# wagnva/semantic-nerf-for-satellite-data

Measured on AMD Instinct MI355X. Metric: train rays/sec (4096 rays x 64 samples), higher is better.
Workload: dtype f32(f16x2)

## Files before the change

### semantic-nerf-for-satellite-data_amd/csrc/api.hip

```cpp
#include <stdarg.h>
#include <stdio.h>
#include <stdlib.h>
#include <string.h>

#include <mutex>

#include "aux_kernels.h"
#include "bsp.h"
#include "composite.h"
#include "gemm.h"
#include "plan.h"

namespace snerf {

int forward_bsp(const Plan& p, const float* pk, const SnerfInputs* in, const SnerfOutputs* out, void* workspace, hipStream_t st);
int backward_bsp(const Plan& p, const float* pk, const SnerfInputs* in, const SnerfOutGrads* go, float* gp, float* d_t, float* d_t_s,
                 void* workspace, hipStream_t st);

static thread_local char g_err[512] = "";
void set_error(const char* fmt, ...) {
  va_list ap;
  va_start(ap, fmt);
  vsnprintf(g_err, sizeof(g_err), fmt, ap);
  va_end(ap);
// ... 179 lines not shown
    p.k_tr[i] = (i == 0) ? p.Ep : (((p.skip_mask >> i) & 1u) ? p.Ep + p.W : p.W);
    p.w_tr[i] = take((size_t)p.W * p.k_tr[i]);
    p.b_tr[i] = take(p.W);
  }
  p.w_fs = take((size_t)(p.W + NARROW) * p.W); p.b_fs = take(p.W + NARROW);
  p.w_h1 = take((size_t)p.N1 * p.FA); p.b_h1 = take(p.N1);
  p.w_s2 = take((size_t)p.H * p.H); p.b_s2 = take(p.H);
  p.w_s3 = take((size_t)p.H * p.H); p.b_s3 = take(p.H);
  p.w_s4 = take((size_t)NARROW * p.H); p.b_s4 = take(NARROW);
  p.w_fin = take((size_t)NARROW * p.KF); p.b_fin = take(NARROW);
  p.sky_floats = 9 * p.H + 4;
  p.sky = take(p.sky_floats);
  p.n_fp32 = off;
  {
    const char* ev = getenv("SNERF_COMPOSE_FEATS");
    p.compose_feats = p.pl == 2 && (p.H & 31) == 0 && p.N1 + NARROW <= 2048 && !(ev && ev[0] == '0' && ev[1] == 0);
  }
  if (!p.compose_feats) { plan_weights(p); plan_bsp(p); return SNERF_OK; }
  Plan q = p;
  q.compose_feats = false;
  plan_weights(q);
  plan_bsp(q);
  plan_weights(p);
  plan_bsp(p);
  if (q.packed_floats > p.packed_floats) p.packed_floats = q.packed_floats;
  if (q.ws_bytes > p.ws_bytes) p.ws_bytes = q.ws_bytes;
  return SNERF_OK;
}

struct TableBuilder {
  CopyTable tabs[4];
  int nt = 0;
  bool missing = false;
  TableBuilder() { memset(tabs, 0, sizeof(tabs)); nt = 1; }
  void add(float* user, int user_ld, int rows, int cols, size_t dst_off, int dst_ld) {
    if (!user) { missing = true; return; }
    if (tabs[nt - 1].n == COPY_TABLE_MAX) ++nt;
    CopyEntry& e = tabs[nt - 1].e[tabs[nt - 1].n++];
    e.user = user; e.user_ld = user_ld; e.rows = rows; e.cols = cols; e.dst_off = dst_off; e.dst_ld = dst_ld;
  }
};

static void build_tables(const Plan& p, const SnerfParams* w, TableBuilder& tb) {
  const int W = p.W, H = p.H, E = p.E;
  for (int i = 0; i < p.L; ++i) {
    const bool skip = (p.skip_mask >> i) & 1u;
    if (i == 0) {
// ... 195 lines not shown
```

### semantic-nerf-for-satellite-data_amd/csrc/aux_kernels.h

```cpp
#pragma once
#include "common.h"
#include "../../include/snerf_hip.h"

namespace snerf {

struct EncodeArgs {
  const float* rays = nullptr;
  const float* xyz = nullptr;
  const float* z = nullptr;
  const float* sun_d = nullptr; int sun_stride = 3;
  const float* t = nullptr; const float* t_s = nullptr;
  int dir_is_sun = 0;
  int N = 0, S = 0, F = 0, Ep = 0;
  int FA = 0, W = 0, Xp = 0, x_sun = 0, x_t = 3, x_ts = -1, tau = 0;
  unsigned* zero = nullptr; int zero_n = 0;
};

struct CopyEntry {
  float* user; int user_ld; int rows; int cols; unsigned long long dst_off; int dst_ld;
};
constexpr int COPY_TABLE_MAX = 40;
struct CopyTable { CopyEntry e[COPY_TABLE_MAX]; int n; };

int launch_zero_bytes(void* p, size_t bytes, hipStream_t st);
int launch_sample_z(const float* rays, const float* zsteps, const float* u, float* z, int N, int S, hipStream_t st);
int launch_copy_table(const CopyTable& tb, float* packed, int mode, hipStream_t st);
int launch_reduce_rows(const float* in, int n_in, size_t in_stride, int width, float* out, size_t out_stride,
                       int group, int accumulate, hipStream_t st);
int reduce_partials(const float* in, int n_in, size_t in_stride, int width, float* tmp, float* out, hipStream_t st);
struct RedJob { const float* in; float* out; unsigned long long stride; long long width; int n_in; int blk0; int vec; int cols; int in_ld; int out_ld; int store; int pad; };
constexpr int RED_MAX = 56;
struct RedTable { RedJob j[RED_MAX]; int n = 0; int blocks = 0; };
constexpr int RED_CHUNK = 24;
struct RedChunk { RedJob j[RED_CHUNK]; int n = 0; };
int red_add_elem(RedTable& tb, const float* in, int n_in, size_t stride, size_t width, float* out);
int red_add_elem2d(RedTable& tb, const float* in, int n_in, size_t stride, int rows, int cols, int in_ld, float* out, int out_ld);
int red_add_col(RedTable& tb, const float* in, int n_in, size_t stride, int width, float* out);
int red_store_last(RedTable& tb);
int launch_reductions(const RedTable& elem, const RedTable& col, hipStream_t st);
// ... 6 lines not shown
```

### semantic-nerf-for-satellite-data_amd/csrc/bsp.h

```cpp
#pragma once
#include "common.h"
#include "gemm.h"

namespace snerf {
namespace bsp {

constexpr int RB = 128;
constexpr int CB = 128;
constexpr int E_MAX = 100;
constexpr int E_QUIET = 60;

typedef __amdgpu_buffer_rsrc_t srd_t;
typedef unsigned int u32x4 __attribute__((ext_vector_type(4)));
typedef unsigned int u32x2 __attribute__((ext_vector_type(2)));
typedef _Float16 f16x8 __attribute__((ext_vector_type(8)));
typedef _Float16 f16x4 __attribute__((ext_vector_type(4)));
constexpr unsigned OOB = 0xFFFFFFF0u;

__host__ __device__ inline int ncb_of(int ld) { return (ld + CB - 1) / CB; }
__host__ __device__ inline size_t plane_bytes(size_t rows, int ld, int pl = 2) { return rows * (size_t)ld * 2 * pl; }
__host__ __device__ inline size_t etab_ints(size_t rows, int ld) { return ((rows + RB - 1) / RB) * (size_t)ncb_of(ld); }
__host__ __device__ inline unsigned g16_off(int k, int pl = 2) { return (unsigned)(k >> 4) * 32u * (unsigned)pl + (unsigned)(k & 15) * 2u; }

__host__ __device__ inline int exp_of_maxbits(unsigned b) {
// ... 65 lines not shown
  int Ka = 0;
  const char* W = nullptr;
  const int* EW = nullptr;
  int w_rb32 = 0, w_row0 = 0, w_k0 = 0; unsigned w_bytes = 0;
  int I = 0, J = 0, K = 0;
  char* C = nullptr; int* EC = nullptr; int ldc = 0; int c_col0 = 0;
  float* Cf = nullptr;
  const float* bias = nullptr;
  int act = ACT_NONE; float w0 = 1.f;
  unsigned* Csign = nullptr;
  int aux_mode = AUX_NONE;
  const char* H = nullptr; const int* EH = nullptr; int ldh = 0; int h_col0 = 0; const unsigned* Hsign = nullptr;
  float* colsum = nullptr; int ldcs = 0;
  int tiles_i = 0, tiles_j = 0;
  int tj_skip = -1;
  int tiles_jr = 0;
  int rev = 0;
  int dbg = 0;
  int* tile_ctr = nullptr;
  int pl = 2;
  const float* nd_w = nullptr; float* nd_out = nullptr; unsigned long long nd_stride = 0;
  int nd_omax = 0, nd_ldw = 0;
  int nd_rows[8] = {0, 0, 0, 0, 0, 0, 0, 0}, nd_row0[8] = {0, 0, 0, 0, 0, 0, 0, 0}, nd_woff[8] = {0, 0, 0, 0, 0, 0, 0, 0};
};
__host__ __device__ inline size_t sign_words(size_t rows, int ld) { return ((rows + 31) / 32) * (size_t)((ld + 63) / 64) * 64; }

struct DwArgs {
  const char* A = nullptr; const int* EA = nullptr; int lda = 0; int a_col0 = 0;
  const char* B = nullptr; const int* EB = nullptr; int ldb = 0; int b_col0 = 0;
  int I = 0, J = 0, P = 0;
  float* C = nullptr; int ldc = 0;
  int k_split = 0, n_split = 1; unsigned long long slab_stride = 0;
  int tiles_i = 0, tiles_j = 0;
  int pl = 2;
};

constexpr int TR_MAXL = 8;
constexpr int TR_SLOTS = TR_MAXL + 1;
struct TrunkArgs {
  const char* pe = nullptr; const int* Epe = nullptr;
  int P = 0, W = 0, L = 0; unsigned skip_mask = 0;
  int gamma_free_layer = 0;
  const char* Wp[TR_SLOTS] = {}; const int* EW[TR_SLOTS] = {}; unsigned w_bytes[TR_SLOTS] = {}; int K[TR_SLOTS] = {};
  const float* bias[TR_SLOTS] = {}; float w0[TR_SLOTS] = {};
  char* F = nullptr; int* EF = nullptr; int ldf = 0;
  char* H[TR_MAXL] = {}; int* EH[TR_MAXL] = {}; unsigned* Hsign[TR_MAXL] = {};
// ... 68 lines not shown
```

### semantic-nerf-for-satellite-data_amd/csrc/bsp_aux.hip

```cpp
#include "bsp.h"
#include "aux_kernels.h"

namespace snerf {
namespace bsp {

__device__ __forceinline__ float block_max_256(float m, float* sm) {
#pragma unroll
  for (int o = 32; o >= 1; o >>= 1) m = fmaxf(m, __shfl_xor(m, o, 64));
  __syncthreads();
  if ((threadIdx.x & 63) == 0) sm[threadIdx.x >> 6] = m;
  __syncthreads();
  return fmaxf(fmaxf(sm[0], sm[1]), fmaxf(sm[2], sm[3]));
}

__global__ __launch_bounds__(256) void to_planes_kernel(const float* __restrict__ src, int ld_src, int rows, int cols,
                                                        char* __restrict__ dst, int* __restrict__ E, int ld, int col0, int pl) {
  __shared__ float sm[4];
  const int rb = blockIdx.y, cb = blockIdx.x;
  const int t = threadIdx.x, c8 = cb * 128 + (t & 15) * 8;
  float v[8][8];
  float m = 0.f;
#pragma unroll
  for (int i = 0; i < 8; ++i) {
    const int r = rb * 128 + (t >> 4) + 16 * i;
// ... 319 lines not shown
#pragma unroll
    for (int half = 0; half < 2; ++half) {
#pragma unroll
      for (int j = 0; j < 8; ++j) h8[j] = v[8 * half + j];
      split8(h8, sc, hi, lo);
      *reinterpret_cast<u32x4*>(d + 16 * half) = hi;
      if (g.pl == 2) *reinterpret_cast<u32x4*>(d + 32 + 16 * half) = lo;
    }
  }
}

int launch_encode_bsp(const EncodeArgs& a, char* pe, int* Epe, char* fa, int* Efa, int fa_col0, int pl, hipStream_t st) {
  if (a.Ep > 128 || (a.Ep & 15) || (fa && ((fa_col0 & 127) || (a.FA & 15) || a.Xp != 16))) {
    set_error("encode: Ep <= 128, Ep % 16 == 0, extras block of 16 columns at a multiple of 128");
    return SNERF_ERR_BAD_DESC;
  }
  EncodeBsp g{a, pe, Epe, fa, Efa, fa_col0, pl};
  const long long P = (long long)a.N * a.S;
  hipLaunchKernelGGL(encode_bsp_kernel, dim3((unsigned)((P + 127) / 128)), dim3(256), 0, st, g);
  SNERF_LAUNCH_CHECK();
  return SNERF_OK;
}

__global__ __launch_bounds__(256) void colsum32_bsp_kernel(const float* __restrict__ in, int rows, float* __restrict__ partial,
                                                           char* __restrict__ pl, int* __restrict__ E, int npl) {
  __shared__ float4 sm[32][8];
  __shared__ float smx[2][2];
  const int c4 = threadIdx.x & 7, rg = threadIdx.x >> 3;
  const int r0 = blockIdx.x * 256;
  float4 v[8];
  float4 s = make_float4(0.f, 0.f, 0.f, 0.f);
  float m[2] = {0.f, 0.f};
#pragma unroll
  for (int i = 0; i < 8; ++i) {
    const int r = r0 + rg + 32 * i;
    v[i] = r < rows ? *reinterpret_cast<const float4*>(in + (size_t)r * 32 + 4 * c4) : make_float4(0.f, 0.f, 0.f, 0.f);
    s.x += v[i].x; s.y += v[i].y; s.z += v[i].z; s.w += v[i].w;
    m[i >> 2] = fmaxf(fmaxf(m[i >> 2], fmaxf(fabsf(v[i].x), fabsf(v[i].y))), fmaxf(fabsf(v[i].z), fabsf(v[i].w)));
  }
  sm[rg][c4] = s;
#pragma unroll
  for (int h = 0; h < 2; ++h) {
#pragma unroll
    for (int o = 32; o >= 1; o >>= 1) m[h] = fmaxf(m[h], __shfl_xor(m[h], o, 64));
  }
  __syncthreads();
// ... 44 lines not shown
```

### semantic-nerf-for-satellite-data_amd/csrc/bsp_kc.hip

```cpp
#include "bsp_kc_epi.h"

namespace snerf {
namespace bsp {

constexpr int KC_A = 128 * 128, KC_RING = 3;
constexpr int KC_RINGB = KC_RING * KC_A;
constexpr int KC_XREG = KC_RINGB;
constexpr int KC_BIAS = KC_XREG + 4 * 4096;
constexpr int KC_ETAB = KC_BIAS + 2 * 1024;
constexpr int KC_SMAX = KC_ETAB + 2 * 512;
constexpr int KC_NEXT = KC_SMAX + 64;
constexpr int KC_HSIGN = KC_NEXT + 64;
constexpr int KC_LDS = KC_HSIGN + 4 * 1024;
constexpr int KC_NDW = KC_HSIGN;
constexpr int KC_NDW_FLOATS = 2560;
constexpr int KC_LDS_ND = KC_NDW + 4 * KC_NDW_FLOATS;
template <int PL, int ACT, int AUX, bool COLSUM, bool SIGNS, int SINM, bool DIAG = false, int NDOT = 0>
__global__ __launch_bounds__(256, 2) void gemm_kc_kernel(const KcArgs) {
  const kargs_t p = kargs();
  __shared__ __attribute__((aligned(16))) char lds[NDOT > 0 ? KC_LDS_ND : KC_LDS];
  float* smax = reinterpret_cast<float*>(lds + KC_SMAX);
  const int t = threadIdx.x, lane = t & 63;
  const int wave = __builtin_amdgcn_readfirstlane(t >> 6);
  const int wj0 = wave * 64;
  const int tiles_i = p->tiles_i, tiles_j = p->tiles_j, ntiles = tiles_i * tiles_j;
  constexpr int EB = 2 * PL;
  constexpr int KSUB = PL == 2 ? 16 : 32, KSH = PL == 2 ? 4 : 5;
  const int nks16 = p->K >> 4;
  const int nks = (p->K + KSUB - 1) >> KSH;
  const int nks1 = p->Ka < p->K ? p->Ka >> KSH : nks;
  const int eW = *p->EW;
  const int nst = (nks + 1) >> 1, nst1 = nks1 >> 1;
  constexpr bool ONEPASS = ACT == ACT_SIN;
  constexpr bool BIAS = AUX == AUX_NONE && !COLSUM;
  const int dbg = DIAG ? p->dbg : 0;

  auto a_lane_off = [&](int q, int ld, int l) -> unsigned {
    const int row = 8 * (wave + 4 * q) + (l >> 3);
    return (unsigned)row * (unsigned)ld * (unsigned)EB + 16u * (unsigned)((l & 7) ^ ((row >> 1) & 7));
  };
// ... 400 lines not shown
      if (AUX == AUX_SINREC) {
        const srd_words srdS = make_srd_words(e->Hsign, clamp_bytes(sign_words((size_t)e->I, e->ldh) * 4ull));
        const unsigned sreg0 = __builtin_amdgcn_readfirstlane(lds_addr(lds + KC_HSIGN + wave * 1024));
#pragma unroll
        for (int mi = 0; mi < 4; ++mi) {
          const bool ok = wave_cols && 32 * mi < nrows;
          const unsigned vo = ok ? (unsigned)((((size_t)((c_i0 >> 5) + mi) * ((e->ldh + 63) >> 6) + ((e->h_col0 + jw) >> 6)) * 64 + el) * 4) : OOBH;
          dma4_asm(srdS, sreg0 + (unsigned)(mi * 256), vo, 0u);
        }
      }
      dma_h(0);
      dma_h(1);
      if constexpr (AUX != AUX_NONE) next_heads();
      const float fac = AUX == AUX_SINREC ? inv_in * fabsf(e->w0) * inv_h : inv_in;
      const int eHc = eH < -60 ? -60 : (eH > 60 ? 60 : eH);
      const float one_s = pow2f(2 * eHc);
      const unsigned sflip = e->w0 < 0.f ? 0xFFFFFFFFu : 0u;
      unsigned sword[4] = {0u, 0u, 0u, 0u};
#pragma unroll
      for (int nj = 0; nj < 2; ++nj) {
        float cs[16];
#pragma unroll
        for (int r = 0; r < 16; ++r) cs[r] = 0.f;
#pragma unroll
        for (int mi = 0; mi < 4; ++mi) {
          const int hb = 4 * nj + mi;
          u32x4 hh[2], hl[2];
          if (AUX != AUX_NONE) {
            if (hb == 7) wait_vm<0>(); else if (hb < 2 && more) wait_vm<HPC + 8>(); else wait_vm<HPC>();
            const char* hreg = (hb & 1) ? lds + KC_XREG + wave * 4096 : lds + 2 * KC_A + wave * 4096;
            if (AUX == AUX_SINREC && nj == 0) sword[mi] = *reinterpret_cast<const unsigned*>(lds + KC_HSIGN + wave * 1024 + mi * 256 + el * 4) ^ sflip;
#pragma unroll
            for (int gg = 0; gg < 2; ++gg) {
              if constexpr (PL == 2) {
                hh[gg] = *reinterpret_cast<const u32x4*>(hreg + pt * 128 + 16 * ((4 * gg + lh) ^ ((pt >> 1) & 7)));
                if (AUX == AUX_SINREC) hl[gg] = *reinterpret_cast<const u32x4*>(hreg + pt * 128 + 16 * ((4 * gg + 2 + lh) ^ ((pt >> 1) & 7)));
              } else {
                hh[gg] = *reinterpret_cast<const u32x4*>(hreg + pt * 64 + 16 * ((2 * gg + lh) ^ ((pt >> 2) & 3)));
              }
            }
            if (hb + 2 < 8) {
              if constexpr (PL == 2 && AUX == AUX_SINREC) asm volatile("s_waitcnt lgkmcnt(0)" : "+v"(hh[0]), "+v"(hh[1]), "+v"(hl[0]), "+v"(hl[1]), "+v"(sword[mi])::"memory");
              else asm volatile("s_waitcnt lgkmcnt(0)" : "+v"(hh[0]), "+v"(hh[1]), "+v"(sword[mi])::"memory");
              dma_h(hb + 2);
            }
          }
// ... 16 lines not shown
#pragma unroll
              for (int c = 0; c < 8; ++c) {
                const float om = fmaf(-sv[c], sv[c], one_s);
                const float root = __builtin_amdgcn_sqrtf(fabsf(om));
                const unsigned rs = __float_as_uint(root) | ((sword[mi] << (31 - (16 * nj + 8 * gg + c))) & 0x80000000u);
                v[c] *= __uint_as_float(rs);
              }
            } else if (AUX == AUX_RELU_MASK) {
              float hv[8];
              cvt8f(hh[gg], hv);
#pragma unroll
              for (int c = 0; c < 8; ++c) v[c] = hv[c] > 0.f ? v[c] : 0.f;
            }
#pragma unroll
            for (int c = 0; c < 8; ++c) {
              if (COLSUM) cs[8 * gg + c] += v[c];
              acc[mi][nj][8 * gg + c] = v[c];
            }
            if (jw + 16 * gq < e->J) {
              const float m8 = absmax3(v[6], v[7], absmax3(v[4], v[5], absmax3(v[2], v[3], absmax3(v[0], v[1], 0.f))));
              wmax = fmaxf(wmax, (BIAS && (32 * mi + pt) >= nrows) ? 0.f : m8);
            }
          }
        }
        if (COLSUM && e->colsum != nullptr) {
#pragma unroll
          for (int r = 0; r < 16; ++r) cs[r] = sum32(cs[r]);
          if ((el & 31) == 31) {
#pragma unroll
            for (int gg = 0; gg < 2; ++gg)
              if (jw + 16 * (2 * nj + gg) < e->J) {
                float* d = e->colsum + (size_t)c_ti * e->ldcs + jw + 16 * (2 * nj + gg) + 8 * lh;
                *reinterpret_cast<float4*>(d) = make_float4(cs[8 * gg] * fac, cs[8 * gg + 1] * fac, cs[8 * gg + 2] * fac, cs[8 * gg + 3] * fac);
                *reinterpret_cast<float4*>(d + 4) = make_float4(cs[8 * gg + 4] * fac, cs[8 * gg + 5] * fac, cs[8 * gg + 6] * fac, cs[8 * gg + 7] * fac);
              }
          }
        }
      }
      constexpr bool RAW = AUX != AUX_NONE || COLSUM;
      wmax = wave_max(wmax) * (RAW ? fac : 1.f);
      if (el == 0) smax[wave] = wmax;
      barrier_raw();
      const float bmax = fmaxf(smax[wave & 2], smax[(wave & 2) + 1]);
      const int eC = exp_of_maxbits(__float_as_uint(bmax));
      const float sc = pow2f(eC) * (RAW ? fac : 1.f);
      if ((wave & 1) == 0 && el == 0 && wave_cols) e->EC[(size_t)c_ti * ncb_of(e->ldc) + ((e->c_col0 + jw) >> 7)] = eC;
      if (more) headW();
#pragma unroll
// ... 39 lines not shown
static int g_kc_grid_override = 0;
void kc_set_grid_override(int n) { g_kc_grid_override = n > 0 ? n : 0; }
static int kc_slots() {
  if (g_kc_grid_override > 0) return g_kc_grid_override;
  static const int n = [] {
    int dev = 0, cus = 256;
    if (hipGetDevice(&dev) != hipSuccess || hipDeviceGetAttribute(&cus, hipDeviceAttributeMultiprocessorCount, dev) != hipSuccess || cus <= 0) cus = 256;
    return 2 * cus;
  }();
  return n;
}

static bool cs_bias_check(const KcArgs& a) {
  if (a.colsum != nullptr && a.bias != nullptr) { set_error("bsp gemm: bias and column sums in one launch"); return true; }
  return false;
}

int launch_kc(const KcArgs& a0, hipStream_t st) {
  KcArgs a = a0;
  if (!a.A2) { a.A2 = a.A; a.EA2 = a.EA; a.lda2 = a.lda; a.a2_col0 = a.a_col0; if (a.Ka == 0) a.Ka = a.K; }
  int rc = check_kc(a, false);
  if (rc) return rc;
  if (cs_bias_check(a)) return SNERF_ERR_BAD_DESC;
  a.tiles_i = (a.I + 127) / 128;
  a.tiles_jr = (a.J + 255) / 256;
  if (a.tj_skip >= a.tiles_jr || (a.tj_skip >= 0 && a.tiles_jr < 2)) { set_error("bsp gemm: tj_skip beyond the column tiles"); return SNERF_ERR_BAD_DESC; }
  a.tiles_j = a.tiles_jr - (a.tj_skip >= 0 ? 1 : 0);
  if (a.nd_w != nullptr) {
    if (a.nd_omax == 0) { a.nd_omax = 1; a.nd_ldw = 0; for (int tj = 0; tj < 8; ++tj) { a.nd_rows[tj] = tj < a.tiles_jr ? 1 : 0; a.nd_row0[tj] = 0; } }
    int off = 0;
    for (int tj = 0; tj < a.tiles_jr && tj < 8; ++tj) { a.nd_woff[tj] = off; off += 256 * a.nd_rows[tj]; }
    if (a.tiles_jr > 8 || off > KC_NDW_FLOATS || (a.nd_omax != 1 && a.nd_omax != 5)) { set_error("bsp gemm: folded projections beyond the LDS table"); return SNERF_ERR_BAD_DESC; }
    for (int tj = 0; tj < a.tiles_jr; ++tj) if (a.nd_rows[tj] > a.nd_omax) { set_error("bsp gemm: nd_rows > nd_omax"); return SNERF_ERR_BAD_DESC; }
  }
#ifdef KC_DIAG_BUILD
  constexpr bool DIAG = true;
  static const int dbg = [] { const char* e = getenv("SNERF_KC_DBG"); return e ? atoi(e) : 0; }();
  a.dbg = dbg;
  if (dbg & 2) a.w_bytes = 0;
#else
  constexpr bool DIAG = false;
#endif
  const int ntiles = a.tiles_i * a.tiles_j, slots = kc_slots();
  const dim3 grid(ntiles < slots ? ntiles : slots), block(256);
  const int tok = prof_hook_begin(2.0 * a.I * (double)a.J * a.K, 0, st);
  const bool cs = a.colsum != nullptr;
#define KC_LAUNCH(ACT_, AUX_, CS_, SG_, SM_) do { if (a.pl == 2) hipLaunchKernelGGL((gemm_kc_kernel<2, ACT_, AUX_, CS_, SG_, SM_, DIAG>), grid, block, 0, st, a); \
                                                 else hipLaunchKernelGGL((gemm_kc_kernel<1, ACT_, AUX_, CS_, SG_, SM_, DIAG>), grid, block, 0, st, a); } while (0)
#define KC_LAUNCH_ND(SG_, ND_) do { if (a.pl == 2) hipLaunchKernelGGL((gemm_kc_kernel<2, ACT_SIN, AUX_NONE, false, SG_, SIN_DIRECT, DIAG, ND_>), grid, block, 0, st, a); \
                                    else hipLaunchKernelGGL((gemm_kc_kernel<1, ACT_SIN, AUX_NONE, false, SG_, SIN_DIRECT, DIAG, ND_>), grid, block, 0, st, a); } while (0)
  if (a.aux_mode == AUX_SINREC) KC_LAUNCH(ACT_NONE, AUX_SINREC, true, false, SIN_FRACT);
  else if (a.aux_mode == AUX_RELU_MASK) KC_LAUNCH(ACT_NONE, AUX_RELU_MASK, true, false, SIN_FRACT);
  else if (a.act == ACT_SIN) {
    if (a.nd_w != nullptr && a.nd_omax == 1) { if (a.Csign == nullptr) KC_LAUNCH_ND(false, 1); else KC_LAUNCH_ND(true, 1); }
    else if (a.nd_w != nullptr) { if (a.Csign == nullptr) KC_LAUNCH_ND(false, 5); else KC_LAUNCH_ND(true, 5); }
    else if (a.Csign == nullptr) KC_LAUNCH(ACT_SIN, AUX_NONE, false, false, SIN_DIRECT);
    else KC_LAUNCH(ACT_SIN, AUX_NONE, false, true, SIN_DIRECT);
  }
  else if (a.act == ACT_RELU) KC_LAUNCH(ACT_RELU, AUX_NONE, false, false, SIN_FRACT);
  else if (cs) KC_LAUNCH(ACT_NONE, AUX_NONE, true, false, SIN_FRACT);
  else KC_LAUNCH(ACT_NONE, AUX_NONE, false, false, SIN_FRACT);
#undef KC_LAUNCH
#undef KC_LAUNCH_ND
  SNERF_LAUNCH_CHECK();
  prof_hook_end(tok, st);
  return SNERF_OK;
}

}
}
```

### semantic-nerf-for-satellite-data_amd/csrc/bsp_pass.hip

```cpp
#include "aux_kernels.h"
#include "bsp.h"
#include "composite.h"
#include "plan.h"

namespace snerf {

namespace {
struct Ws {
  char* base;
  char* c(size_t off) const { return base + off; }
  float* f(size_t off) const { return reinterpret_cast<float*>(base + off); }
  int* i(size_t off) const { return reinterpret_cast<int*>(base + off); }
  unsigned* u(size_t off) const { return reinterpret_cast<unsigned*>(base + off); }
  void a(bsp::KcArgs& g, const PlaneT& t, int k, int col0 = 0) const { g.A = c(t.o); g.EA = i(t.e); g.lda = t.ld; g.a_col0 = col0; g.Ka = k; }
  void a2(bsp::KcArgs& g, const PlaneT& t) const { g.A2 = c(t.o); g.EA2 = i(t.e); g.lda2 = t.ld; }
  void out(bsp::KcArgs& g, const PlaneT& t, int col0 = 0) const { g.C = c(t.o); g.EC = i(t.e); g.ldc = t.ld; g.c_col0 = col0; g.Csign = t.s ? u(t.s) : nullptr; }
  void h(bsp::KcArgs& g, const PlaneT& t, int col0 = 0) const { g.H = c(t.o); g.EH = i(t.e); g.ldh = t.ld; g.h_col0 = col0; g.Hsign = t.s ? u(t.s) : nullptr; }
  void dz(bsp::DwArgs& g, const PlaneT& t) const { g.A = c(t.o); g.EA = i(t.e); g.lda = t.ld; g.a_col0 = 0; }
  void x(bsp::DwArgs& g, const PlaneT& t, int col0) const { g.B = c(t.o); g.EB = i(t.e); g.ldb = t.ld; g.b_col0 = col0; }
};
struct WOp { const char* W; const int* EW; int rb32; unsigned bytes; int K; };
WOp wop(const Plan& p, const float* pk, int job) {
  const char* planes = reinterpret_cast<const char*>(pk + p.n_fp32);
  const bsp::WPackJob& w = p.wj.j[job];
// ... 133 lines not shown
  if (p.train) { c.save_T = ws.f(p.o_T); c.save_rgbraw = ws.f(p.o_rgbraw); }
  RC(launch_composite_fwd(c, st));
  return SNERF_OK;
}

namespace {
struct RQ {
  float* base; size_t cap, used = 0; bool over = false;
  RedTable elem, col;
  float* take(size_t floats) {
    const size_t n = round_up_sz(floats, 64);
    if (used + n > cap) { over = true; return base; }
    float* r = base ? base + used : nullptr; used += n; return r;
  }
};
struct DwMat { DwSplit sp; size_t stride; int ldw; float* slab; };
inline int cs_ld(int width) { return (width + 3) & ~3; }

struct BwdRegions {
  float *nar_fin = nullptr, *nar_sun = nullptr, *nar_sig = nullptr;
  DwMat w_fin, w_s4, w_s3, w_s2, w_h1, w_fs;
  float *cs_fin = nullptr, *cs_s3 = nullptr, *cs_s2 = nullptr, *cs_sun = nullptr, *cs_fa = nullptr, *cs_hl = nullptr;
  int ld_cs1 = 0;
  struct Layer { DwMat w, w_gamma; float* cs; } tr[SNERF_MAX_LAYERS];
};
void take_regions(const Plan& p, RQ& rq, BwdRegions& r) {
  auto dw = [&](int rows, int ldw, int cols, bool narrow_rows, int split_rows = 0) {
    DwMat m;
    m.sp = dw_choose_bsp(p.P, split_rows > 0 ? split_rows : rows, cols, narrow_rows);
    m.stride = round_up_sz((size_t)rows * ldw, 64);
    m.ldw = ldw;
    m.slab = rq.take(m.stride * m.sp.ns);
    return m;
  };
  auto cs = [&](int width) { return rq.take((size_t)((p.P + 127) / 128) * cs_ld(width)); };
  auto nar = [&]() { return rq.take((size_t)((p.P + 255) / 256) * NARROW); };
  const int W = p.W, H = p.H;
  if (!p.sc) { r.nar_fin = nar(); r.w_fin = dw(NARROW, p.KF, p.KF, true); if (!p.compose_feats) r.cs_fin = cs(p.KF); }
  r.nar_sun = nar(); r.w_s4 = dw(NARROW, H, H, true); r.w_s3 = dw(H, H, H, false); r.w_s2 = dw(H, H, H, false);
  r.cs_s3 = cs(H); r.cs_s2 = cs(H);
  if (p.compose_feats) {
    r.ld_cs1 = cs_ld(p.h1w); r.cs_fin = cs(p.h1w); r.cs_sun = r.cs_fin + (p.sc ? 0 : p.sun_col);
    r.w_h1 = dw(p.h1w, p.FA, p.FA, false);
    r.nar_sig = nar(); r.w_fs = dw(NARROW, W, W, false, W); r.cs_hl = cs(W);
  } else {
    r.cs_sun = cs(H);
    r.w_h1 = dw(p.h1w, p.FA, p.FA, false); r.cs_fa = cs(p.FA);
    r.nar_sig = nar(); r.w_fs = dw(W + NARROW, W, W, false, W); r.cs_hl = cs(W);
  }
  for (int i = p.L - 1; i >= 0; --i) {
    if (i > 0 && ((p.skip_mask >> i) & 1u)) { r.tr[i].w_gamma = dw(W, p.Ep, p.Ep, false); r.tr[i].w = dw(W, W, W, false); }
    else r.tr[i].w = dw(W, p.k_tr[i], i == 0 ? p.Ep : W, false);
    r.tr[i].cs = i > 0 ? cs(W) : nullptr;
  }
}
}

size_t bsp_rq_floats(const Plan& p) {
  RQ rq{nullptr, ~(size_t)0};
  BwdRegions r;
  take_regions(p, rq, r);
  return rq.used;
}

int backward_bsp(const Plan& p, const float* pk, const SnerfInputs* in, const SnerfOutGrads* go, float* gp, float* d_t, float* d_t_s,
                 void* workspace, hipStream_t st) {
// ... 34 lines not shown
  c.sun_d = in->sun_d; c.sun_stride = in->sun_stride; c.sky = pk + p.sky;
  b.T = ws.f(p.o_T); b.rgbraw = ws.f(p.o_rgbraw);
  b.g_rgb = go->rgb; b.g_depth = go->depth; b.g_weights = go->weights; b.g_transparency = go->transparency;
  b.g_albedo = go->albedo; b.g_sun = go->sun; b.g_sky = go->sky; b.g_beta = go->beta; b.g_sigmas = go->sigmas;
  b.g_beta_s = go->beta_semantic; b.g_logits = go->semantic_logits;
  b.d_sigo = dsig; b.d_fino = dfin; b.d_suno = dsun; b.sky_slab = p.sc ? nullptr : ws.f(p.o_skyslab);
  b.zero = ws.u(p.o_kcq); b.zero_n = KCQ_SLOTS * 16;
  RC(launch_composite_bwd(b, st));
  if (!p.sc)
    RC(red_add_col(rq.col, ws.f(p.o_skyslab), p.comp_blocks * 4, (size_t)p.sky_floats, p.sky_floats, gp + p.sky));


  const PlaneT dz1 = p.dza.view(p.h1w);
  const int sun_col = p.sc ? 0 : p.sun_col;
  if (!p.sc) {
    RC(narrow_grad(dfin, r.nar_fin, p.pdfin, gp + p.b_fin));
    RC(dw_gemm(r.w_fin, p.pdfin, NARROW, true, p.h1, 0, p.KF));
    RC(dw_reduce(r.w_fin, (size_t)NARROW * p.KF, gp + p.w_fin));
    bsp::KcArgs g;
    ws.a(g, p.pdfin, NARROW); weights(g, p, pk, p.wj_tfin);
    g.I = P; g.J = p.KF; g.K = NARROW; ws.out(g, dz1);
    dact(g, p.h1);
    colsum(g, r.cs_fin, p.KF);
    if (p.compose_feats) g.ldcs = r.ld_cs1;
    RC(launch_kc(g));
    if (!p.compose_feats) RC(bias_from_colsum(r.cs_fin, p.KF, gp + p.b_h1));
  }
  {
    RC(narrow_grad(dsun, r.nar_sun, p.pdsun, gp + p.b_s4));
    RC(dw_gemm(r.w_s4, p.pdsun, NARROW, true, p.s3, 0, H));
    RC(dw_reduce(r.w_s4, (size_t)NARROW * H, gp + p.w_s4));
    bsp::KcArgs g;
    ws.a(g, p.pdsun, NARROW); weights(g, p, pk, p.wj_ts4);
    g.I = P; g.J = H; g.K = NARROW; ws.out(g, p.dsa);
    dact(g, p.s3);
    colsum(g, r.cs_s3, H);
    RC(launch_kc(g));
    RC(bias_from_colsum(r.cs_s3, H, gp + p.b_s3));
    RC(dw_gemm(r.w_s3, p.dsa, H, false, p.s2, 0, H));
    RC(dw_reduce(r.w_s3, (size_t)H * H, gp + p.w_s3));
    ws.a(g, p.dsa, H); g.K = H; weights(g, p, pk, p.wj_ts3);
    ws.out(g, p.dsb);
    dact(g, p.s2);
    colsum(g, r.cs_s2, H);
    RC(launch_kc(g));
    RC(bias_from_colsum(r.cs_s2, H, gp + p.b_s2));
    RC(dw_gemm(r.w_s2, p.dsb, H, false, p.h1, sun_col, H));
    RC(dw_reduce(r.w_s2, (size_t)H * H, gp + p.w_s2));
    ws.a(g, p.dsb, H); weights(g, p, pk, p.wj_ts2);
    ws.out(g, dz1, sun_col);
    dact(g, p.h1, sun_col);
    colsum(g, r.cs_sun, H);
    if (p.compose_feats) g.ldcs = r.ld_cs1;
    RC(launch_kc(g));
    if (!p.compose_feats) RC(bias_from_colsum(r.cs_sun, H, gp + p.b_h1 + (size_t)p.sun_col));
  }
  auto transient_grads = [&]() {
    const bool want_t = d_t != nullptr, want_ts = d_t_s != nullptr && p.x_ts >= 0;
    if (p.sc) {
      if (want_t) RC(launch_zero_bytes(d_t, (size_t)p.N * p.tau * sizeof(float), st));
      if (want_ts) RC(launch_zero_bytes(d_t_s, (size_t)p.N * p.tau * sizeof(float), st));
    } else if (want_t || want_ts) {
      int b_lo = p.blk_beta, b_hi = p.blk_beta;
      auto use = [&](int blk, bool on) { if (on && blk >= 0) { if (blk < b_lo) b_lo = blk; if (blk > b_hi) b_hi = blk; } };
      use(p.blk_rgb, p.rgb_t); use(p.blk_sem, p.sem_t || p.sem_ts); use(p.blk_sbeta, true);
      const int k_lo = b_lo * H, k_n = (b_hi + 1 - b_lo) * H;
      float* dext = ws.f(p.o_dfin);
      bsp::KcArgs x;
      ws.a(x, dz1, k_n, k_lo); weights(x, p, pk, p.wj_th1, p.Wf, k_lo);
      x.I = P; x.J = p.Xp; x.K = k_n; x.Cf = dext;
      RC(bsp::launch_kc_narrow(x, st));
      if (want_t) RC(launch_ray_sum32(dext, p.x_t, p.N, p.S, p.tau, d_t, st));
      if (want_ts) RC(launch_ray_sum32(dext, p.x_ts, p.N, p.S, p.tau, d_t_s, st));
    }
    return (int)SNERF_OK;
  };
  PlaneT dz_cur = p.dza.view(W);
  PlaneT dz_nxt = p.dzb.view(W);
  const bool sig_live = !p.sc || go->weights != nullptr || go->transparency != nullptr || go->sigmas != nullptr;
  const PlaneT& hl = p.h[p.L - 1];
  bool uncompose = false;
  if (p.compose_feats) {
    const int r0 = p.sc ? p.sun_col : 0;
    const int nt = (P + 127) / 128, X = p.FA - W;
    RC(dw_gemm(r.w_h1, dz1, p.h1w, false, p.fa, 0, p.FA));
    RC(red_add_elem2d(rq.elem, r.w_h1.slab + W, r.w_h1.sp.ns, r.w_h1.stride, p.h1w, X, p.FA, gp + p.w_h1 + (size_t)r0 * p.FA + W, p.FA));
    RC(red_add_elem2d(rq.elem, r.w_h1.slab, r.w_h1.sp.ns, r.w_h1.stride, p.h1w, W, p.FA, r.w_h1.slab, p.FA));
    RC(red_store_last(rq.elem));
    RC(red_add_col(rq.col, r.cs_fin, nt, (size_t)r.ld_cs1, p.h1w, r.cs_fin));
    RC(red_store_last(rq.col));
    uncompose = true;
    RC(transient_grads());
    if (sig_live) {
      RC(narrow_grad(dsig, r.nar_sig, p.pdsig, gp + p.b_fs + W));
      RC(dw_gemm(r.w_fs, p.pdsig, NARROW, true, hl, 0, W));
      RC(dw_reduce(r.w_fs, (size_t)NARROW * W, gp + p.w_fs + (size_t)W * W));
    }
    { const PlaneT sw = dz_cur; dz_cur = dz_nxt; dz_nxt = sw; }
    bsp::KcArgs g;
    ws.a(g, dz1, p.h1w);
    if (sig_live) ws.a2(g, p.pdsig);
    weights(g, p, pk, p.wj_th1, 0, r0); g.I = P; g.J = W; g.K = sig_live ? p.h1w + NARROW : p.h1w;
    ws.out(g, dz_cur);
    dact(g, hl, 0, (p.L == 1) ? 30.f : 1.f);
    colsum(g, r.cs_hl, W);
    RC(launch_kc(g));
    RC(bias_from_colsum(r.cs_hl, W, gp + p.b_tr[p.L - 1]));
  }
  const PlaneT dfa = p.dzb.view(p.FA);
  if (!p.compose_feats) {
    const int r0 = p.sc ? p.sun_col : 0;
    RC(dw_gemm(r.w_h1, dz1, p.h1w, false, p.fa, 0, p.FA));
    RC(dw_reduce(r.w_h1, (size_t)p.h1w * p.FA, gp + p.w_h1 + (size_t)r0 * p.FA));
// ... 58 lines not shown
```

### semantic-nerf-for-satellite-data_amd/csrc/plan.h

```cpp
#pragma once
#include "bsp.h"
#include "common.h"
#include "../../include/snerf_hip.h"

namespace snerf {

constexpr int NARROW = 32;
constexpr int MAX_CLASSES = 16;
constexpr int ND_FIN = 5;
constexpr int MAX_SKY_UNITS = 8;

struct PlaneT { size_t o = 0, e = 0, s = 0; int ld = 0; };
struct PlaneScratch {
  size_t o = 0, e = 0; int maxw = 0;
  PlaneT view(int ld) const { PlaneT t; t.o = o; t.e = e; t.ld = ld; return t; }
};

struct Plan {
  int N = 0, S = 0, P = 0, Pp = 0;
  int W = 0, H = 0, L = 0, E = 0, Ep = 0, F = 0, tau = 0, C = 0;
  bool siren = false, train = false, sc = false, sem_sigmoid = false;
  unsigned skip_mask = 0;
  int x_sun = 0, x_t = 3, x_ts = -1, Xp = 0, FA = 0;
  int nblk = 0, blk_rgb = 0, blk_sem = -1, blk_beta = -1, blk_sbeta = -1, blk_sun = -1;
// ... 17 lines not shown
  size_t packed_floats = 0;
  int pl = 2;

  size_t o_z = 0, o_T = 0, o_rgbraw = 0;
  PlaneT pe, fa, h1, s2, s3, h[SNERF_MAX_LAYERS];
  size_t o_sigo = 0, o_fino = 0, o_suno = 0;
  size_t o_sigpart = 0, o_sunpart = 0, o_finpart = 0;
  bool nd_sig = false, nd_sun = false;
  bool fuse_trunk = false;
  bool nd_fin = false;
  PlaneScratch dza, dzb;
  PlaneT dsa, dsb, pdsig, pdfin, pdsun;
  size_t o_dsig = 0, o_dfin = 0, o_dsun = 0;
  size_t o_skyslab = 0;
  size_t o_kcq = 0;
  size_t o_rq = 0, rq_floats = 0;
  bsp::WPackTable wj = {};
  int wj_tr[SNERF_MAX_LAYERS] = {0}, wj_tt[SNERF_MAX_LAYERS] = {0};
  int wj_fs = 0, wj_sig = 0, wj_tfs = 0, wj_h1 = 0, wj_th1 = 0, wj_s2 = 0, wj_ts2 = 0, wj_s3 = 0, wj_ts3 = 0, wj_s4 = 0, wj_ts4 = 0,
      wj_fin = 0, wj_tfin = 0;
  size_t wp_bytes = 0;
  int h1w = 0;
  bool compose_feats = false;
  int wj_first = 0;
  size_t o_wc = 0;
  size_t o_bc = 0;
  int comp_blocks = 0;
  size_t ws_bytes = 0;
};

constexpr int KCQ_SLOTS = 64;
struct DwSplit { int ns = 1; int k_split = 32; };
DwSplit dw_choose_bsp(int P, int rows, int cols, bool narrow_rows);

#define RC(expr) do { int _rc = (expr); if (_rc) return _rc; } while (0)

int make_plan(const SnerfDesc* d, Plan* pl);

size_t bsp_rq_floats(const Plan& p);

}
```

Before: 170,600.

## Compute per-ray extras weight grads and transient grads from per-block column sums

Adds a ray_extras path. The backward GEMM epilogue emits per-32-row column sums (one row per ray, since S is a multiple of 32), and a new kernel uses these per-ray sums to build the weight gradient for the per-ray extra input columns (sun direction, transient embeddings). The same kernel also produces the transient embedding gradients, which replaces both the wide dW GEMM over those columns and the separate transient GEMM. It relies on the extra inputs being constant within a ray, and it adds workspace, a new kernel and extra column-sum stores. The path falls back when it would need more workspace.

New measurement: 171,600 (median of 6 runs). Within noise of the previous version (+0.6%).

```diff
diff --git a/semantic-nerf-for-satellite-data_amd/csrc/api.hip b/semantic-nerf-for-satellite-data_amd/csrc/api.hip
--- a/semantic-nerf-for-satellite-data_amd/csrc/api.hip
+++ b/semantic-nerf-for-satellite-data_amd/csrc/api.hip
@@ -225,7 +225,12 @@
   plan_weights(q);
   plan_bsp(q);
   plan_weights(p);
+  {
+    const char* ev = getenv("SNERF_RAY_EXTRAS");
+    p.ray_extras = (p.S & 31) == 0 && !(ev && ev[0] == '0' && ev[1] == 0);
+  }
   plan_bsp(p);
+  if (p.ray_extras && p.ws_bytes > q.ws_bytes) { p.ray_extras = false; plan_bsp(p); }
   if (q.packed_floats > p.packed_floats) p.packed_floats = q.packed_floats;
   if (q.ws_bytes > p.ws_bytes) p.ws_bytes = q.ws_bytes;
   return SNERF_OK;
diff --git a/semantic-nerf-for-satellite-data_amd/csrc/aux_kernels.h b/semantic-nerf-for-satellite-data_amd/csrc/aux_kernels.h
--- a/semantic-nerf-for-satellite-data_amd/csrc/aux_kernels.h
+++ b/semantic-nerf-for-satellite-data_amd/csrc/aux_kernels.h
@@ -15,6 +15,22 @@
   int FA = 0, W = 0, Xp = 0, x_sun = 0, x_t = 3, x_ts = -1, tau = 0;
   unsigned* zero = nullptr; int zero_n = 0;
 };
+
+struct RayExtrasArgs {
+  EncodeArgs a;
+  const float* Q = nullptr; int ldq = 0;
+  int h1w = 0;
+  const float* Wx = nullptr; int ldw = 0;
+  int k_lo = 0, k_n = 0;
+  float* slab = nullptr;
+  float* gsum = nullptr;
+  float* part = nullptr;
+  int rays_per_group = 0;
+};
+namespace bsp {
+void ray_extras_grid(int N, int h1w, int& groups, int& rays_per_group, int& chunks);
+int launch_ray_extras(const RayExtrasArgs& a, hipStream_t st);
+}
 
 struct CopyEntry {
   float* user; int user_ld; int rows; int cols; unsigned long long dst_off; int dst_ld;
diff --git a/semantic-nerf-for-satellite-data_amd/csrc/bsp.h b/semantic-nerf-for-satellite-data_amd/csrc/bsp.h
--- a/semantic-nerf-for-satellite-data_amd/csrc/bsp.h
+++ b/semantic-nerf-for-satellite-data_amd/csrc/bsp.h
@@ -111,6 +111,7 @@
   const float* nd_w = nullptr; float* nd_out = nullptr; unsigned long long nd_stride = 0;
   int nd_omax = 0, nd_ldw = 0;
   int nd_rows[8] = {0, 0, 0, 0, 0, 0, 0, 0}, nd_row0[8] = {0, 0, 0, 0, 0, 0, 0, 0}, nd_woff[8] = {0, 0, 0, 0, 0, 0, 0, 0};
+  int cs32 = 0;
 };
 __host__ __device__ inline size_t sign_words(size_t rows, int ld) { return ((rows + 31) / 32) * (size_t)((ld + 63) / 64) * 64; }
 
diff --git a/semantic-nerf-for-satellite-data_amd/csrc/bsp_aux.hip b/semantic-nerf-for-satellite-data_amd/csrc/bsp_aux.hip
--- a/semantic-nerf-for-satellite-data_amd/csrc/bsp_aux.hip
+++ b/semantic-nerf-for-satellite-data_amd/csrc/bsp_aux.hip
@@ -365,6 +365,78 @@
   return SNERF_OK;
 }
 
+__global__ __launch_bounds__(256) void ray_extras_kernel(const RayExtrasArgs g) {
+  __shared__ float Rs[16][257];
+  __shared__ float ws[256][17];
+  __shared__ __attribute__((aligned(16))) float es[16][16];
+  const int t = threadIdx.x, chunk = blockIdx.x, grp = blockIdx.y;
+  const int col = 256 * chunk + t;
+  const bool col_ok = col < g.h1w;
+  const int kb = g.a.S >> 5;
+  const int n0 = grp * g.rays_per_group, n1 = min(g.a.N, n0 + g.rays_per_group);
+  const int j_lo = max(g.k_lo, 256 * chunk) - 256 * chunk, j_hi = min(min(g.k_lo + g.k_n, g.h1w), 256 * chunk + 256) - 256 * chunk;
+  const bool want_d = j_lo < j_hi;
+  if (want_d) {
+#pragma unroll
+    for (int c = 0; c < 16; ++c) ws[t][c] = col_ok ? g.Wx[(size_t)col * g.ldw + c] : 0.f;
+  }
+  float acc[16], gsum = 0.f;
+#pragma unroll
+  for (int c = 0; c < 16; ++c) acc[c] = 0.f;
+  for (int nb = n0; nb < n1; nb += 16) {
+    __syncthreads();
+    { const int n = nb + (t >> 4); es[t >> 4][t & 15] = n < n1 ? extras_value(g.a, n, t & 15) : 0.f; }
+    float R[16];
+#pragma unroll
+    for (int i = 0; i < 16; ++i) R[i] = 0.f;
+    const float* q = g.Q + (size_t)nb * kb * g.ldq + (col_ok ? col : 0);
+    for (int b = 0; b < kb; ++b) {
+      float v[16];
+#pragma unroll
+      for (int i = 0; i < 16; ++i) v[i] = q[((size_t)(nb + i < n1 ? i : 0) * kb + b) * g.ldq];
+#pragma unroll
+      for (int i = 0; i < 16; ++i) R[i] += (col_ok && nb + i < n1) ? v[i] : 0.f;
+    }
+#pragma unroll
+    for (int i = 0; i < 16; ++i) { Rs[i][t] = R[i]; gsum += R[i]; }
+    __syncthreads();
+#pragma unroll
+    for (int i = 0; i < 16; ++i)
+#pragma unroll
+      for (int c = 0; c < 16; ++c) acc[c] = fmaf(R[i], es[i][c], acc[c]);
+    if (want_d) {
+      const int i = t >> 4, c = t & 15;
+      float d = 0.f;
+      for (int j = j_lo; j < j_hi; ++j) d = fmaf(Rs[i][j], ws[j][c], d);
+      if (nb + i < n1) g.part[((size_t)chunk * g.a.N + nb + i) * 16 + c] = d;
+    }
+  }
+  if (col_ok) {
+    float4* o = reinterpret_cast<float4*>(g.slab + ((size_t)grp * g.h1w + col) * 16);
+#pragma unroll
+    for (int c = 0; c < 4; ++c) o[c] = make_float4(acc[4 * c], acc[4 * c + 1], acc[4 * c + 2], acc[4 * c + 3]);
+    g.gsum[(size_t)grp * g.h1w + col] = gsum;
+  }
+}
+void ray_extras_grid(int N, int h1w, int& groups, int& rays_per_group, int& chunks) {
+  groups = (N + 15) / 16 < 64 ? (N + 15) / 16 : 64;
+  rays_per_group = round_up((N + groups - 1) / groups, 16);
+  groups = (N + rays_per_group - 1) / rays_per_group;
+  chunks = (h1w + 255) / 256;
+}
+int launch_ray_extras(const RayExtrasArgs& a, hipStream_t st) {
+  int groups, rpg, chunks;
+  ray_extras_grid(a.a.N, a.h1w, groups, rpg, chunks);
+  if (a.a.N <= 0 || a.a.S <= 0 || (a.a.S & 31) || a.h1w <= 0 || (a.h1w & 15) || a.ldq < a.h1w || rpg != a.rays_per_group || a.k_lo < 0 || a.k_n < 0 ||
+      a.Q == nullptr || a.Wx == nullptr || a.slab == nullptr || a.gsum == nullptr || (a.k_n > 0 && a.part == nullptr) || a.a.sun_d == nullptr) {
+    set_error("ray_extras: S % 32 == 0, h1w % 16 == 0 and the grid of ray_extras_grid are required");
+    return SNERF_ERR_BAD_DESC;
+  }
+  hipLaunchKernelGGL(ray_extras_kernel, dim3(chunks, groups), dim3(256), 0, st, a);
+  SNERF_LAUNCH_CHECK();
+  return SNERF_OK;
+}
+
 __global__ __launch_bounds__(256) void colsum32_bsp_kernel(const float* __restrict__ in, int rows, float* __restrict__ partial,
                                                            char* __restrict__ pl, int* __restrict__ E, int npl) {
   __shared__ float4 sm[32][8];
diff --git a/semantic-nerf-for-satellite-data_amd/csrc/bsp_kc.hip b/semantic-nerf-for-satellite-data_amd/csrc/bsp_kc.hip
--- a/semantic-nerf-for-satellite-data_amd/csrc/bsp_kc.hip
+++ b/semantic-nerf-for-satellite-data_amd/csrc/bsp_kc.hip
@@ -15,7 +15,7 @@
 constexpr int KC_NDW = KC_HSIGN;
 constexpr int KC_NDW_FLOATS = 2560;
 constexpr int KC_LDS_ND = KC_NDW + 4 * KC_NDW_FLOATS;
-template <int PL, int ACT, int AUX, bool COLSUM, bool SIGNS, int SINM, bool DIAG = false, int NDOT = 0>
+template <int PL, int ACT, int AUX, bool COLSUM, bool SIGNS, int SINM, bool DIAG = false, int NDOT = 0, bool CS32 = false>
 __global__ __launch_bounds__(256, 2) void gemm_kc_kernel(const KcArgs) {
   const kargs_t p = kargs();
   __shared__ __attribute__((aligned(16))) char lds[NDOT > 0 ? KC_LDS_ND : KC_LDS];
@@ -462,6 +462,19 @@
         float cs[16];
 #pragma unroll
         for (int r = 0; r < 16; ++r) cs[r] = 0.f;
+        auto cs_emit = [&](int row) {
+#pragma unroll
+          for (int r = 0; r < 16; ++r) cs[r] = sum32(cs[r]);
+          if ((el & 31) == 31) {
+#pragma unroll
+            for (int gg = 0; gg < 2; ++gg)
+              if (jw + 16 * (2 * nj + gg) < e->J) {
+                float* d = e->colsum + (size_t)row * e->ldcs + jw + 16 * (2 * nj + gg) + 8 * lh;
+                *reinterpret_cast<float4*>(d) = make_float4(cs[8 * gg] * fac, cs[8 * gg + 1] * fac, cs[8 * gg + 2] * fac, cs[8 * gg + 3] * fac);
+                *reinterpret_cast<float4*>(d + 4) = make_float4(cs[8 * gg + 4] * fac, cs[8 * gg + 5] * fac, cs[8 * gg + 6] * fac, cs[8 * gg + 7] * fac);
+              }
+          }
+        };
 #pragma unroll
         for (int mi = 0; mi < 4; ++mi) {
           const int hb = 4 * nj + mi;
@@ -524,8 +537,13 @@
               wmax = fmaxf(wmax, (BIAS && (32 * mi + pt) >= nrows) ? 0.f : m8);
             }
           }
-        }
-        if (COLSUM && e->colsum != nullptr) {
+          if constexpr (COLSUM && CS32) {
+            cs_emit(4 * c_ti + mi);
+#pragma unroll
+            for (int r = 0; r < 16; ++r) cs[r] = 0.f;
+          }
+        }
+        if (COLSUM && !CS32 && e->colsum != nullptr) {
 #pragma unroll
           for (int r = 0; r < 16; ++r) cs[r] = sum32(cs[r]);
           if ((el & 31) == 31) {
@@ -611,6 +629,7 @@
   int rc = check_kc(a, false);
   if (rc) return rc;
   if (cs_bias_check(a)) return SNERF_ERR_BAD_DESC;
+  if (a.cs32 && (a.pl != 2 || a.aux_mode == AUX_NONE || a.colsum == nullptr)) { set_error("bsp gemm: per-block column sums need two planes, a derivative epilogue and a partials buffer"); return SNERF_ERR_BAD_DESC; }
   a.tiles_i = (a.I + 127) / 128;
   a.tiles_jr = (a.J + 255) / 256;
   if (a.tj_skip >= a.tiles_jr || (a.tj_skip >= 0 && a.tiles_jr < 2)) { set_error("bsp gemm: tj_skip beyond the column tiles"); return SNERF_ERR_BAD_DESC; }
@@ -638,7 +657,11 @@
                                                  else hipLaunchKernelGGL((gemm_kc_kernel<1, ACT_, AUX_, CS_, SG_, SM_, DIAG>), grid, block, 0, st, a); } while (0)
 #define KC_LAUNCH_ND(SG_, ND_) do { if (a.pl == 2) hipLaunchKernelGGL((gemm_kc_kernel<2, ACT_SIN, AUX_NONE, false, SG_, SIN_DIRECT, DIAG, ND_>), grid, block, 0, st, a); \
                                     else hipLaunchKernelGGL((gemm_kc_kernel<1, ACT_SIN, AUX_NONE, false, SG_, SIN_DIRECT, DIAG, ND_>), grid, block, 0, st, a); } while (0)
-  if (a.aux_mode == AUX_SINREC) KC_LAUNCH(ACT_NONE, AUX_SINREC, true, false, SIN_FRACT);
+  if (a.cs32) {
+    if (a.aux_mode == AUX_SINREC) hipLaunchKernelGGL((gemm_kc_kernel<2, ACT_NONE, AUX_SINREC, true, false, SIN_FRACT, DIAG, 0, true>), grid, block, 0, st, a);
+    else hipLaunchKernelGGL((gemm_kc_kernel<2, ACT_NONE, AUX_RELU_MASK, true, false, SIN_FRACT, DIAG, 0, true>), grid, block, 0, st, a);
+  }
+  else if (a.aux_mode == AUX_SINREC) KC_LAUNCH(ACT_NONE, AUX_SINREC, true, false, SIN_FRACT);
   else if (a.aux_mode == AUX_RELU_MASK) KC_LAUNCH(ACT_NONE, AUX_RELU_MASK, true, false, SIN_FRACT);
   else if (a.act == ACT_SIN) {
     if (a.nd_w != nullptr && a.nd_omax == 1) { if (a.Csign == nullptr) KC_LAUNCH_ND(false, 1); else KC_LAUNCH_ND(true, 1); }
diff --git a/semantic-nerf-for-satellite-data_amd/csrc/bsp_pass.hip b/semantic-nerf-for-satellite-data_amd/csrc/bsp_pass.hip
--- a/semantic-nerf-for-satellite-data_amd/csrc/bsp_pass.hip
+++ b/semantic-nerf-for-satellite-data_amd/csrc/bsp_pass.hip
@@ -179,6 +179,8 @@
   DwMat w_fin, w_s4, w_s3, w_s2, w_h1, w_fs;
   float *cs_fin = nullptr, *cs_s3 = nullptr, *cs_s2 = nullptr, *cs_sun = nullptr, *cs_fa = nullptr, *cs_hl = nullptr;
   int ld_cs1 = 0;
+  float *rx_slab = nullptr, *rx_gsum = nullptr, *rx_part = nullptr;
+  int rx_groups = 0, rx_rpg = 0, rx_chunks = 0;
   struct Layer { DwMat w, w_gamma; float* cs; } tr[SNERF_MAX_LAYERS];
 };
 void take_regions(const Plan& p, RQ& rq, BwdRegions& r) {
@@ -197,8 +199,19 @@
   r.nar_sun = nar(); r.w_s4 = dw(NARROW, H, H, true); r.w_s3 = dw(H, H, H, false); r.w_s2 = dw(H, H, H, false);
   r.cs_s3 = cs(H); r.cs_s2 = cs(H);
   if (p.compose_feats) {
-    r.ld_cs1 = cs_ld(p.h1w); r.cs_fin = cs(p.h1w); r.cs_sun = r.cs_fin + (p.sc ? 0 : p.sun_col);
-    r.w_h1 = dw(p.h1w, p.FA, p.FA, false);
+    r.ld_cs1 = cs_ld(p.h1w);
+    if (p.ray_extras) {
+      r.cs_fin = rq.take((size_t)4 * ((p.P + 127) / 128) * r.ld_cs1);
+      bsp::ray_extras_grid(p.N, p.h1w, r.rx_groups, r.rx_rpg, r.rx_chunks);
+      r.rx_slab = rq.take((size_t)r.rx_groups * p.h1w * 16);
+      r.rx_gsum = rq.take((size_t)r.rx_groups * p.h1w);
+      if (!p.sc) r.rx_part = rq.take((size_t)r.rx_chunks * p.N * 16);
+      r.w_h1 = dw(p.h1w, p.FA, W, false);
+    } else {
+      r.cs_fin = cs(p.h1w);
+      r.w_h1 = dw(p.h1w, p.FA, p.FA, false);
+    }
+    r.cs_sun = r.cs_fin + (p.sc ? 0 : p.sun_col);
     r.nar_sig = nar(); r.w_fs = dw(NARROW, W, W, false, W); r.cs_hl = cs(W);
   } else {
     r.cs_sun = cs(H);
@@ -279,7 +292,7 @@
     g.I = P; g.J = p.KF; g.K = NARROW; ws.out(g, dz1);
     dact(g, p.h1);
     colsum(g, r.cs_fin, p.KF);
-    if (p.compose_feats) g.ldcs = r.ld_cs1;
+    if (p.compose_feats) { g.ldcs = r.ld_cs1; g.cs32 = p.ray_extras ? 1 : 0; }
     RC(launch_kc(g));
     if (!p.compose_feats) RC(bias_from_colsum(r.cs_fin, p.KF, gp + p.b_h1));
   }
@@ -308,20 +321,30 @@
     ws.out(g, dz1, sun_col);
     dact(g, p.h1, sun_col);
     colsum(g, r.cs_sun, H);
-    if (p.compose_feats) g.ldcs = r.ld_cs1;
+    if (p.compose_feats) { g.ldcs = r.ld_cs1; g.cs32 = p.ray_extras ? 1 : 0; }
     RC(launch_kc(g));
     if (!p.compose_feats) RC(bias_from_colsum(r.cs_sun, H, gp + p.b_h1 + (size_t)p.sun_col));
   }
+  const bool want_t = d_t != nullptr, want_ts = d_t_s != nullptr && p.x_ts >= 0;
+  int k_lo = 0, k_n = 0;
+  if (!p.sc && (want_t || want_ts)) {
+    int b_lo = p.blk_beta, b_hi = p.blk_beta;
+    auto use = [&](int blk, bool on) { if (on && blk >= 0) { if (blk < b_lo) b_lo = blk; if (blk > b_hi) b_hi = blk; } };
+    use(p.blk_rgb, p.rgb_t); use(p.blk_sem, p.sem_t || p.sem_ts); use(p.blk_sbeta, true);
+    k_lo = b_lo * H; k_n = (b_hi + 1 - b_lo) * H;
+  }
   auto transient_grads = [&]() {
-    const bool want_t = d_t != nullptr, want_ts = d_t_s != nullptr && p.x_ts >= 0;
     if (p.sc) {
       if (want_t) RC(launch_zero_bytes(d_t, (size_t)p.N * p.tau * sizeof(float), st));
       if (want_ts) RC(launch_zero_bytes(d_t_s, (size_t)p.N * p.tau * sizeof(float), st));
+    } else if (p.ray_extras) {
+      if (k_n > 0) {
+        const int ch_lo = k_lo / 256, n_ch = (k_lo + k_n - 1) / 256 + 1 - ch_lo;
+        const float* part = r.rx_part + (size_t)ch_lo * p.N * 16;
+        if (want_t) { RC(red_add_elem2d(rq.elem, part + p.x_t, n_ch, (size_t)p.N * 16, p.N, p.tau, 16, d_t, p.tau)); RC(red_store_last(rq.elem)); }
+        if (want_ts) { RC(red_add_elem2d(rq.elem, part + p.x_ts, n_ch, (size_t)p.N * 16, p.N, p.tau, 16, d_t_s, p.tau)); RC(red_store_last(rq.elem)); }
+      }
     } else if (want_t || want_ts) {
-      int b_lo = p.blk_beta, b_hi = p.blk_beta;
-      auto use = [&](int blk, bool on) { if (on && blk >= 0) { if (blk < b_lo) b_lo = blk; if (blk > b_hi) b_hi = blk; } };
-      use(p.blk_rgb, p.rgb_t); use(p.blk_sem, p.sem_t || p.sem_ts); use(p.blk_sbeta, true);
-      const int k_lo = b_lo * H, k_n = (b_hi + 1 - b_lo) * H;
       float* dext = ws.f(p.o_dfin);
       bsp::KcArgs x;
       ws.a(x, dz1, k_n, k_lo); weights(x, p, pk, p.wj_th1, p.Wf, k_lo);
@@ -340,12 +363,30 @@
   if (p.compose_feats) {
     const int r0 = p.sc ? p.sun_col : 0;
     const int nt = (P + 127) / 128, X = p.FA - W;
-    RC(dw_gemm(r.w_h1, dz1, p.h1w, false, p.fa, 0, p.FA));
-    RC(red_add_elem2d(rq.elem, r.w_h1.slab + W, r.w_h1.sp.ns, r.w_h1.stride, p.h1w, X, p.FA, gp + p.w_h1 + (size_t)r0 * p.FA + W, p.FA));
+    if (p.ray_extras) {
+      RC(dw_gemm(r.w_h1, dz1, p.h1w, false, p.fa, 0, W));
+      RayExtrasArgs x;
+      x.a.N = p.N; x.a.S = p.S; x.a.sun_d = in->sun_d; x.a.sun_stride = in->sun_stride; x.a.t = in->t; x.a.t_s = in->t_s;
+      x.a.x_sun = p.x_sun; x.a.x_t = p.x_t; x.a.x_ts = p.x_ts; x.a.tau = p.tau;
+      x.Q = r.cs_fin; x.ldq = r.ld_cs1; x.h1w = p.h1w;
+      x.Wx = pk + p.w_h1 + (size_t)r0 * p.FA + p.Wf; x.ldw = p.FA;
+      x.k_lo = k_lo; x.k_n = k_n;
+      x.slab = r.rx_slab; x.gsum = r.rx_gsum; x.part = r.rx_part; x.rays_per_group = r.rx_rpg;
+      RC(bsp::launch_ray_extras(x, st));
+      RC(red_add_elem2d(rq.elem, r.rx_slab, r.rx_groups, (size_t)p.h1w * 16, p.h1w, 16, 16, gp + p.w_h1 + (size_t)r0 * p.FA + p.Wf, p.FA));
+    } else {
+      RC(dw_gemm(r.w_h1, dz1, p.h1w, false, p.fa, 0, p.FA));
+      RC(red_add_elem2d(rq.elem, r.w_h1.slab + W, r.w_h1.sp.ns, r.w_h1.stride, p.h1w, X, p.FA, gp + p.w_h1 + (size_t)r0 * p.FA + W, p.FA));
+    }
     RC(red_add_elem2d(rq.elem, r.w_h1.slab, r.w_h1.sp.ns, r.w_h1.stride, p.h1w, W, p.FA, r.w_h1.slab, p.FA));
     RC(red_store_last(rq.elem));
-    RC(red_add_col(rq.col, r.cs_fin, nt, (size_t)r.ld_cs1, p.h1w, r.cs_fin));
-    RC(red_store_last(rq.col));
+    if (p.ray_extras) {
+      RC(red_add_elem(rq.elem, r.rx_gsum, r.rx_groups, (size_t)p.h1w, (size_t)p.h1w, r.cs_fin));
+      RC(red_store_last(rq.elem));
+    } else {
+      RC(red_add_col(rq.col, r.cs_fin, nt, (size_t)r.ld_cs1, p.h1w, r.cs_fin));
+      RC(red_store_last(rq.col));
+    }
     uncompose = true;
     RC(transient_grads());
     if (sig_live) {
diff --git a/semantic-nerf-for-satellite-data_amd/csrc/plan.h b/semantic-nerf-for-satellite-data_amd/csrc/plan.h
--- a/semantic-nerf-for-satellite-data_amd/csrc/plan.h
+++ b/semantic-nerf-for-satellite-data_amd/csrc/plan.h
@@ -63,6 +63,7 @@
   size_t wp_bytes = 0;
   int h1w = 0;
   bool compose_feats = false;
+  bool ray_extras = false;
   int wj_first = 0;
   size_t o_wc = 0;
   size_t o_bc = 0;
```
